# alexnodeland/fugue

Measured on AMD Instinct MI355X. Metric: hmc_leapfrog_steps_per_sec, higher is better.
Workload: dtype f64; 1 GPU; C2-normal32: hmc_chain, 32-site conjugate Normal (x#i~N(0,1), y#i~N(x#i,0.5)=0.2i-1), 65536 chains/GPU, L=16, HMCConfig::default; chains_per_gpu=65536, chains_total=65536, n_leapfrog=16, transitions_per_launch=25

## Files before the change

fugue_amd/build.py:

```python
from __future__ import annotations

import hashlib
import os
import subprocess
import sys
from concurrent.futures import ThreadPoolExecutor

HERE = os.path.dirname(os.path.abspath(__file__))
CSRC = os.path.join(HERE, "csrc")
LIB_DIR = os.path.join(HERE, "lib")
LIB = os.environ.get("FG_LIB_PATH") or os.path.join(LIB_DIR, "libfugue_amd.so")
OBJ_DIR = os.path.join(LIB_DIR, "obj")
SOURCES = ["fg_program.cpp", "fg_dsl.cpp", "fg_diag_host.cpp", "fg_jit.cpp", "fg_engine.hip", "fg_hmc_sep.hip", "fg_hmc_lin.hip", "fg_hmc_interp.hip", "fg_mh.hip", "fg_mh_interp.hip", "fg_smc.hip", "fg_diag.hip", "fg_diag_stream.hip", "fg_diag_qstream.hip", "fg_diag_cstream.hip", "fg_loglik_stream.hip", "fg_state.hip", "fg_vi.hip", "fg_result.hip", "fg_predict.hip", "fg_abc.hip", "fg_rng_debug.hip"]
HEADERS = ["fg_ir.h", "fg_math.h", "fg_interp.h", "fg_program.h", "fg_engine_internal.h", "fg_diag_internal.h", "fg_gradstream.h", "fg_cold.h", "fg_dev_types.h", "fg_jit.h",
           "fg_switch.h", "fg_div2.h", "fg_hmc_sep_plan.h", "fg_mh_mw_plan.h", "fg_hmc_split_plan.h", "fg_diag_qstream_plan.h", "fg_diag_cstream_plan.h", "fg_loglik_stream_plan.h", "fg_result_plan.h", "fg_predict_plan.h", "fg_abc_plan.h", "fg_smc_plan.h", "fg_hmc_jit_body.h", "fg_mh_interp_body.h", "fg_mh_mw_body.h", "fg_mh_mw2_body.h",
           os.path.join("..", "..", "include", "fugue_amd.h")]
FLAGS = ["-O3", "-std=c++17", "-fPIC", "--offload-arch=gfx950", "-ffp-contract=off", "-fno-fast-math", "-DFG_BUILD", "-Wall",
         "-Wno-unused-function"]
LINK_LIBS = []


JIT_HEAD = ["fg_ir.h", "fg_math.h", "fg_cold.h", "fg_dev_types.h"]
JIT_BODIES = {"FG_JIT_EMBED_HMC_BODY": "fg_hmc_jit_body.h", "FG_JIT_EMBED_MH_BODY": "fg_mh_interp_body.h", "FG_JIT_EMBED_INTERP": "fg_interp.h",
              "FG_JIT_EMBED_GRADSTREAM": "fg_gradstream.h", "FG_JIT_EMBED_MHMW_BODY": "fg_mh_mw_body.h", "FG_JIT_EMBED_MHMW2_BODY": "fg_mh_mw2_body.h",
              "FG_JIT_EMBED_API": os.path.join("..", "..", "include", "fugue_amd.h")}


def _write_jit_embed():
    def text(name):
        lines = open(os.path.join(CSRC, name)).read().splitlines()
# ... 127 lines not shown
```

fugue_amd/csrc/fg_dev_types.h:

```cpp
#pragma once
#include "fg_ir.h"

struct FgChainCtx {
    long long C;
    uint32_t chain0;
    unsigned long long seed;
    long long *values;
    double *gtile;
    int gtile_rows;
};


struct FgHmcDev {
    double *lj, *eps, *frozen, *da_mu, *da_leb, *da_hbar;
    unsigned long long *da_m;
    double *m_inv, *mass_sqrt, *w_mean, *w_m2;
    unsigned long long *w_n;
    double *alpha_sum; unsigned long long *n_div;
    double *p0_scratch;
    int L; double h, target; int grad_mode; int use_mass;
    double div2_hi, div2_lo; int div2;
};


__device__ __forceinline__ double fg_kinetic(const FgProgramDev &P, const double *pl, int tw, const double *m_inv, long long C) {
    double s = 0.0;
    if (m_inv) {
        for (int i = 0; i < P.d; ++i) { const double p = pl[i * tw]; s += p * p * m_inv[(long long)i * C]; }
    } else {
#pragma unroll 8
        for (int i = 0; i < P.d; ++i) { const double p = pl[i * tw]; s += p * p; }
    }
    return 0.5 * s;
}


// ... 44 lines not shown
```

fugue_amd/csrc/fg_engine.hip:

```cpp
#include "fg_engine_internal.h"
#include "fg_hmc_sep_plan.h"
#include "fg_div2.h"
#include "fg_gradstream.h"
#include "fg_cold.h"

template <bool GT>
__global__ __launch_bounds__(FG_WAVE, FG_MIN_WAVES) void k_prior_init(FgProgramDev P, FgChainCtx X, uint32_t iteration, uint32_t purpose,
                                                        double *acc_out , double *lj_out ) {
    extern __shared__ double lds_[];
    double *lds = GT ? X.gtile + (size_t)blockIdx.x * X.gtile_rows * FG_WAVE : lds_;
    constexpr int tw = FG_WAVE;
    const long long chain = (long long)blockIdx.x * tw + threadIdx.x;
    const bool live = chain < X.C;
    const long long c = live ? chain : X.C - 1;
    double *slots = lds + threadIdx.x;
    for (int j = 0; j < P.n_slots; ++j) slots[j * tw] = 0.0;
    FgStream rng = fg_stream(X.seed, X.chain0 + (uint32_t)c, iteration, purpose);
    FgAcc3 A = {0.0, 0.0, 0.0};
    fg_exec<FG_MODE_PRIOR, false>(P.ins, P.n_ins, P.pool, slots, tw, A, &rng, nullptr, 0, live);
    if (live) {
        fg_store_values(P, X, c, slots, tw);
        if (acc_out) { acc_out[c] = A.prior; acc_out[X.C + c] = A.lik; acc_out[2 * X.C + c] = A.fac; }
        if (lj_out) lj_out[c] = fg_total(A);
    }
// ... 809 lines not shown
            return FG_E_HIP;
    }
    if (mass && !e->H.m_inv) {
        if (A(&e->H.m_inv, d * C) || A(&e->H.mass_sqrt, d * C) || A(&e->H.w_mean, d * C) || A(&e->H.w_m2, d * C) || A(&e->H.w_n, C))
            return FG_E_HIP;
    }
    return FG_OK;
}

void fg_internal_hmc_set_cfg(fg_engine *e, const fg_hmc_config *cfg) {
    e->cfg = *cfg;
    e->H.L = cfg->n_leapfrog > 1 ? cfg->n_leapfrog : 1;
    e->H.h = cfg->finite_diff_eps; e->H.target = cfg->target_accept;
    e->H.grad_mode = cfg->grad_mode;
    e->H.div2 = fg_div2_prove(2.0 * e->H.h, &e->H.div2_hi, &e->H.div2_lo) ? 1 : 0;
}

static bool hmc_jit_first(const fg_engine *e) {
    const FgJitFirstIn in = { e->cfg.grad_mode, e->jit_state, e->P.gstream != nullptr, e->gt, e->tw, fg_hmc_sep_gate(e->gt, e->P.sep != nullptr, e->sep_disabled, e->d), fg_hmc_lin_gate(e) };
    return fg_hmc_jit_first(in);
}

static int hmc_find_eps(fg_engine *e, uint32_t instance, int injected, double *d_eps_out) {
    if (hmc_jit_first(e)) {
        const int rc = fg_hmc_jit_find_eps(e, instance, injected, d_eps_out);
        if (rc != FG_E_UNSUPPORTED) return rc;
    }
    FG_LAUNCH_GT(e, k_hmc_find_eps, dim3((unsigned)((e->C + e->tw - 1) / e->tw)), dim3(e->tw), e->lds_bytes, e->stream, e->P, e->X, e->H, instance,
                       injected, d_eps_out);
    HIPCHK(hipGetLastError());
// ... 228 lines not shown
    HIPCHK(hipGetLastError());
    e->n_warmup = std::min(e->n_warmup, e->iter);
    if (e->mass_adapt_at >= e->iter) e->mass_adapt_at = -1;
    return FG_OK;
}
int fg_hmc_set_n_leapfrog(fg_engine *e, int n_leapfrog) {
    NEED_ENGINE(e);
    if (!e->hmc_ready) return FG_E_STATE;
    e->cfg.n_leapfrog = n_leapfrog > 1 ? n_leapfrog : 1;
    e->H.L = e->cfg.n_leapfrog;
    return FG_OK;
}
const char *fg_hmc_last_kernel(const fg_engine *e) { return e ? e->last_hmc_kernel.c_str() : ""; }
const char *fg_mh_last_kernel(const fg_engine *e) { return e ? e->last_mh_kernel.c_str() : ""; }
int fg_hmc_short_quotient(const fg_engine *e) { return (e && e->hmc_ready && e->H.div2) ? 1 : 0; }
int fg_hmc_is_warming_up(const fg_engine *e) { return (e && e->hmc_ready && e->iter < e->n_warmup) ? 1 : 0; }
int64_t fg_hmc_iterations(const fg_engine *e) { return (e && e->hmc_ready) ? (int64_t)e->iter : 0; }

int fg_hmc_grad(fg_engine *e, double h, int grad_mode, double *h_grad, int32_t *h_ok) {
    NEED_ENGINE(e);
    if (!h_grad) return FG_E_BAD_ARG;
    if (int rc = hmc_lds_ok(e)) return rc;
    if (grad_mode == FG_GRAD_ANALYTIC && (!e->P.gstream || fg_program_stream_records(e->prog, 2) > 1)) {
        fg_set_error("FG_GRAD_ANALYTIC is not available for this program"); return FG_E_UNSUPPORTED; }
    double *d_g = nullptr;
    int rc = dev_alloc(&d_g, (size_t)std::max(1, e->d) * e->C);
    if (rc) return rc;
    FG_LAUNCH_GT(e, k_hmc_grad, dim3((unsigned)((e->C + e->tw - 1) / e->tw)), dim3(e->tw), e->lds_bytes, e->stream, e->P, e->X, h,
                       grad_mode == FG_GRAD_ANALYTIC ? 2 : (grad_mode == FG_GRAD_FD_SPARSE ? 1 : 0), d_g, e->d_itmp);
    hipError_t le = hipGetLastError();
// ... 213 lines not shown
```

fugue_amd/csrc/fg_hmc_sep.hip:

```cpp
#include "fg_engine_internal.h"
#include "fg_gradstream.h"
#define FG_COLD_UKEY 1
#include "fg_cold.h"
#include "fg_hmc_sep_plan.h"

static_assert(FG_SEP_WAVE == FG_WAVE, "fg_hmc_sep_plan.h sizes tiles for 64-lane waves");

#ifdef FG_HMC_PROF
__device__ unsigned long long fg_hmc_prof[FG_SEP_WMAX][8];
#define FG_PROF_T(i) { const unsigned long long now_ = __builtin_readcyclecounter(); prof_[i] += now_ - tprev_; tprev_ = now_; }
#else
#define FG_PROF_T(i)
#endif
#ifndef FG_SEP_STAGGER
#define FG_SEP_STAGGER 2
#endif

__device__ __forceinline__ fg_u32x8 fg_sep_ld8(const FG_AS4 char *p) { return *(const FG_AS4 fg_u32x8 *)p; }
__device__ __forceinline__ fg_u32x4 fg_sep_ld4(const FG_AS4 char *p) { return *(const FG_AS4 fg_u32x4 *)p; }
__device__ __forceinline__ fg_u32x8 fg_sep_ld8(const char *p) { return *(const fg_u32x8 *)p; }
__device__ __forceinline__ fg_u32x4 fg_sep_ld4(const char *p) { return *(const fg_u32x4 *)p; }
#define FG_SEP_LOAD(k) \
    const fg_u32x8 a##k = fg_sep_ld8(rb + 64 * k); \
    const fg_u32x4 b##k = fg_sep_ld4(rb + 64 * k + 32);
// ... 20 lines not shown
    { const double c = fg_dbl(a##k[2], a##k[3]); const double zp = FG_SEP_Z(k, qp - c), zm = FG_SEP_Z(k, qm - c); \
      outp = FG_SEP_LPF(k, zp); outm = FG_SEP_LPF(k, zm); }
#define FG_SEP_DUALS(k, outp, outm)                                                                    \
    double outp, outm;                                                                                 \
    { const double c = fg_dbl(a##k[2], a##k[3]); const double dp = qp - c, dm = qm - c;                \
      outp = __builtin_fma(nhs2_##k, dp * dp, -fg_dbl(a##k[6], a##k[7])) - 0.5 * FG_LN_2PI;            \
      outm = __builtin_fma(nhs2_##k, dm * dm, -fg_dbl(a##k[6], a##k[7])) - 0.5 * FG_LN_2PI; }
#define FG_SEPD_OWN(k, outp, outm) double outp, outm;                                                  \
    { const double c_ = fg_dbl(a##k[2], a##k[3]); const double zp_ = FG_SEP_Z(k, qp - c_), zm_ = FG_SEP_Z(k, qm - c_); \
      const double lp_ = FG_SEP_LP(k, zp_), lm_ = FG_SEP_LP(k, zm_);                                    \
      outp = (zp_ != zp_) ? FG_NEG_INF : lp_; outm = (zm_ != zm_) ? FG_NEG_INF : lm_; }

template <typename RB> struct FgSepScalarRb { static constexpr bool value = false; };
template <> struct FgSepScalarRb<const FG_AS4 char *> { static constexpr bool value = true; };

template <int NOBS, bool P2, bool CHECK, bool AN = false, bool U0 = false, bool FOLD = false, typename RB = const FG_AS4 char *>
__device__ __forceinline__ bool fg_sep_trajectory(RB rb, double &q_io, double &p_io, double emi, double hk, int L, double h, double two_h,
                                                  double rcp_2h, double *terms, int tw, int nobs_rt, double c_hi = 0.0, double c_lo = 0.0) {
#define FG_SEP_HAS(k) (NOBS >= 0 ? NOBS >= (k) : nobs_rt >= (k))
    FG_SEP_LOAD(0) FG_SEP_LOAD(1) FG_SEP_LOAD(2) FG_SEP_LOAD(3)
    double q = q_io, p = p_io;
    bool bad = false;
    constexpr bool FOLDED = FOLD && P2 && !CHECK && !AN;
    double nhs2_0 = 0.0, nhs2_1 = 0.0, nhs2_2 = 0.0, nhs2_3 = 0.0;
#define FG_SEP_NHS2(k) if (FOLDED && (k > 0 || !U0) && FG_SEP_HAS(k)) { nhs2_##k = fg_dbl(b##k[2], b##k[3]); asm volatile("" : "+v"(nhs2_##k)); }
    FG_SEP_NHS2(0) FG_SEP_NHS2(1) FG_SEP_NHS2(2) FG_SEP_NHS2(3)
#undef FG_SEP_NHS2
    if (FOLD && !CHECK && !AN && FgSepScalarRb<RB>::value) asm volatile("" : "+s"(h), "+s"(c_hi), "+s"(c_lo));
    uint32_t nrange = 0u;
    for (int gs = 0; gs <= L; ++gs) {
        double g;
        if (AN) {
#define FG_SEP_ANTERM(k) { const double dl = q - fg_dbl(a##k[2], a##k[3]);                                                   \
        const double w = (P2 || (a##k[0] & FG_G_POW2)) ? (dl * fg_dbl(a##k[4], a##k[5])) * fg_dbl(a##k[4], a##k[5])         \
                                                       : (dl / fg_dbl(b##k[0], b##k[1])) / fg_dbl(b##k[0], b##k[1]); g = g - w; }
            g = 0.0;
            FG_SEP_ANTERM(0)
            if (FG_SEP_HAS(1)) FG_SEP_ANTERM(1)
            if (FG_SEP_HAS(2)) FG_SEP_ANTERM(2)
            if (FG_SEP_HAS(3)) FG_SEP_ANTERM(3)
#undef FG_SEP_ANTERM
        } else {
        const double qp = q + h, qm = q - h;
        double tp, tm;
        if (FOLDED) {
// ... 18 lines not shown
            }
        } else {
        if (U0) { tp = FG_SEP_LP_U(qp); tm = FG_SEP_LP_U(qm); }
        else { FG_SEP_DUAL(0, tp_, tm_) tp = tp_; tm = tm_; }
        if (FG_SEP_HAS(1)) {
            FG_SEP_DUAL(1, lp1, lm1)
            double sp = lp1, sm = lm1;
            if (FG_SEP_HAS(2)) { FG_SEP_DUAL(2, lp2, lm2) sp += lp2; sm += lm2; }
            if (FG_SEP_HAS(3)) { FG_SEP_DUAL(3, lp3, lm3) sp += lp3; sm += lm3; }
            tp = tp + sp; tm = tm + sm;
        }
        }
        const double n = tp - tm;
        if (!CHECK && FOLD) g = __builtin_fma(n, c_hi, n * c_lo);
        else g = fg_div_const(n, two_h, rcp_2h);
        if (!CHECK && FOLD) {
            uint32_t hi = (uint32_t)__double2hiint(n);
            asm("" : "+v"(hi));
            const uint32_t nr = (hi << 1) - 0x19000000u;
            nrange = nrange > nr ? nrange : nr;
        } else {
        const double an = __builtin_fabs(n);
        if (__builtin_expect(__any(!(an >= 0x1p-823 && an <= 0x1p953)), 0)) g = n / two_h;
        }
        }
        if (CHECK) bad = bad || !fg_finite(g);
        const double kick = hk * g;
        p = p + kick;
        if (gs > 0 && gs < L) { asm volatile(""); p = p + kick; }
        if (gs < L) { asm volatile(""); q = q + emi * p; }
    }
    if (!CHECK && FOLD && nrange >= 0xde000000u) p = __builtin_nan("");
    if (U0) { double lp = FG_SEP_LP_U(q); FG_SEP_NAN_NEG_INF(q, lp) terms[a0[1] * tw] = lp; }
    else FG_SEP_TERM(0)
    if (FG_SEP_HAS(1)) FG_SEP_TERM(1)
    if (FG_SEP_HAS(2)) FG_SEP_TERM(2)
    if (FG_SEP_HAS(3)) FG_SEP_TERM(3)
    q_io = q; p_io = p;
    return bad;
#undef FG_SEP_HAS
}

template <bool AN, typename RB>
__device__ __noinline__ FgD3 fg_sep_trajectory_checked(RB rb, double q, double p, double emi, double hk, int L, double h,
                                                       double two_h, double rcp_2h, double *terms, int tw, int nobs) {
    const bool bad = fg_sep_trajectory<-1, false, true, AN, false, false, RB>(rb, q, p, emi, hk, L, h, two_h, rcp_2h, terms, tw, nobs);
    FgD3 r; r.a = q; r.b = p; r.c = bad ? 1.0 : 0.0;
// ... 95 lines not shown
            double pj = p[j] + hk * g;
            if (gs > 0 && gs < L) pj = pj + hk * g;
            p[j] = pj;
            if (gs < L) q[j] = q[j] + (MASS ? e * mii[j] : e) * pj;
        }
    }
#pragma unroll
    for (int j = 0; j < NC; ++j) {
        if (live) H.p0_scratch[(long long)ci[j] * X.C + c] = q[j];
        kin0[(long long)ci[j] * tw] = k0v[j];
        kin1[(long long)ci[j] * tw] = MASS ? p[j] * p[j] * mii[j] : p[j] * p[j];
    }
    return bad;
}

template <bool MASS, int MODE, int HALF = 0 , int NC = 0, int NOBS_R = 0, bool U0_R = false, bool FOLD = false>
__global__ __launch_bounds__(FG_WAVE * FG_SEP_WMAX, 4) void k_hmc_sep_steps(FgProgramDev P, FgChainCtx X, FgHmcDev H, FgSegSep seg, int iter0, int n_steps,
                                                                             int n_warmup, int welford_on, double *draws, int first_sample_t,
                                                                             double *pos_all , double *info ) {
    extern __shared__ double lds[];
    constexpr int tw = FG_WAVE >> HALF;
    constexpr bool DFAST = MODE == 3, DENSE = MODE == 1 || DFAST, AN = MODE == 2;
    static_assert(!HALF || MODE == 0, "half tiles: sparse finite difference only");
    constexpr bool RES = NC > 0;
    constexpr int NCX = RES ? NC : 1;
    static_assert(!RES || (MODE == 0 && HALF == 0 && NC <= 4 && NOBS_R >= 0 && NOBS_R <= 3), "resident form: sparse 64-chain tiles");
    static_assert(!FOLD || MODE == 0, "the folded trajectory loop: sparse finite difference only");
    const int lane = threadIdx.x & (tw - 1);
    const int half = HALF == 1 ? (int)((threadIdx.x >> 5) & 1u) : (HALF == 2 ? (int)((threadIdx.x >> 4) & 3u) : 0);
    const int wv = __builtin_amdgcn_readfirstlane((int)(threadIdx.x >> 6));
    const long long chain = (long long)blockIdx.x * tw + lane;
    const bool live = chain < X.C;
    const bool live0 = live && half == 0;
    const long long c = live ? chain : X.C - 1;
    const int d = P.d, L = H.L, n_s = P.n_sstream, n_pri = P.n_prior_terms;
    const int srows = P.n_sep_free > 0 ? P.n_slots : 0;
    double *slots = lds + lane;
    double *terms = lds + (long long)(srows + (DENSE ? 0 : 2 * d)) * tw + lane;
    double *xch = terms + (long long)n_s * tw;
    double *qrow = xch + 3 * tw, *prow = qrow + (long long)d * tw;
    double *kin0 = DENSE ? qrow : lds + (long long)srows * tw + lane;
    double *kin1 = DENSE ? prow : kin0 + (long long)d * tw;
// ... 71 lines not shown
#pragma unroll
            for (int j = 0; j < NCX; ++j) {
                if (j >= nown) break;
                const int i = k0 + j;
                if (prio_turns) { if ((j ^ (wv >> 2)) & 1) __builtin_amdgcn_s_setprio(1); else __builtin_amdgcn_s_setprio(0); }
                double z;
                if (!(j & 1)) { const FgD2 zz = have_pre ? zn[j >> 1] : fg_cold_normal_pair(sk0, sk1, gchain, (uint32_t)(i >> 1), (uint32_t)iter, FG_RNG_HMC); z = zz.a; zb = zz.b; }
                else z = zb;
                double p = MASS ? z * msr[j] : z;
                const double mii = mir[j];
                kin0R[i * tw] = MASS ? p * p * mii : p * p;
                double q = qc[j];
                const double emi = MASS ? e * mii : e;
                const double q0 = q, p0 = p;
                const FG_AS4 char *rb = (const FG_AS4 char *)(uintptr_t)(P.sep + roff[j]);
                fg_sep_trajectory<NOBS_R, true, false, false, U0_R, FOLD>(rb, q, p, emi, hk, L, h, two_h, rcp_2h, termsR, tw, NOBS_R, c_hi, c_lo);
                if (__builtin_expect(__any(!fg_finite(p)), 0)) {
                    q = q0; p = p0;
                    FG_SEP_2H(th, rc)
                    bad = fg_sep_trajectory<NOBS_R, true, true, false, U0_R>(rb, q, p, emi, hk, L, h, th, rc, termsR, tw, NOBS_R) || bad;
                }
                qpr[j] = q;
                kin1R[i * tw] = MASS ? p * p * mii : p * p;
            }
        } else if (DFAST) {
            const int own[4] = { seg.own[wv][0], seg.own[wv][1], seg.own[wv][2], seg.own[wv][3] };
#define FG_DENSE_CALL(NC_, OBS_) fg_dense_trajectory<NC_, OBS_, MASS>(P, X, H, own, terms, qrow, kin0, kin1, tw, n_pri, n_s, L, e, h, two_h, rcp_2h, sk0, sk1, gchain, (uint32_t)iter, c, live)
            const int nown = seg.n_own[wv];
            if (n_s > n_pri) { if (nown == 4) bad = FG_DENSE_CALL(4, true); else if (nown == 3) bad = FG_DENSE_CALL(3, true); else if (nown == 2) bad = FG_DENSE_CALL(2, true); else bad = FG_DENSE_CALL(1, true); }
            else { if (nown == 4) bad = FG_DENSE_CALL(4, false); else if (nown == 3) bad = FG_DENSE_CALL(3, false); else if (nown == 2) bad = FG_DENSE_CALL(2, false); else bad = FG_DENSE_CALL(1, false); }
#undef FG_DENSE_CALL
// ... 101 lines not shown
                }
            }
            else if (!(i & 1)) { const FgD2 zz = (HALF != 0 && i == k0 && have_pre) ? zpre : fg_cold_normal_pair(sk0, sk1, gchain, (uint32_t)(i >> 1), (uint32_t)iter, FG_RNG_HMC); z = zz.a; zb = zz.b; }
            else z = zb;
            double p = MASS ? z * ms[(long long)ci * X.C] : z;
            const double mii = MASS ? mi[(long long)ci * X.C] : 1.0;
            if (on) kin0[ci * tw] = MASS ? p * p * mii : p * p;
            const long long gq = (long long)P.f64_site[ci] * X.C + c;
            double q = fg_as_double(X.values[gq]);
            const double emi = MASS ? e * mii : e;
            const FgSepCoord cd = P.sep_coord[i];
            const int nobs = (cd.n & 7) - 1;
            const double q0 = q, p0 = p;
            if (HALF) {
                const char *rb = (const char *)(P.sep + P.sep_coord[ci].off);
#define FG_SEP_CALLH(NO, UU) fg_sep_trajectory<NO, true, false, false, UU, FOLD, const char *>(rb, q, p, emi, hk, L, h, two_h, rcp_2h, terms, tw, NO, c_hi, c_lo)
                if ((cd.n & 512) && nobs == 1) FG_SEP_CALLH(1, true);
                else if (nobs == 1) FG_SEP_CALLH(1, false); else if (nobs == 0) FG_SEP_CALLH(0, false); else if (nobs == 2) FG_SEP_CALLH(2, false); else FG_SEP_CALLH(3, false);
#undef FG_SEP_CALLH
                if (__builtin_expect(__any(!fg_finite(p)), 0)) {
                    FG_SEP_2H(th, rc)
                    const FgD3 r = fg_sep_trajectory_checked<AN, const char *>(rb, q0, p0, emi, hk, L, h, th, rc, terms, tw, nobs);
                    q = r.a; p = r.b; bad = bad || (on && r.c != 0.0);
                }
            } else {
            const FG_AS4 char *rb = (const FG_AS4 char *)(uintptr_t)(P.sep + cd.off);
#define FG_SEP_CALL(NO, PP) fg_sep_trajectory<NO, PP, false, AN, false, FOLD>(rb, q, p, emi, hk, L, h, two_h, rcp_2h, terms, tw, NO, c_hi, c_lo)
            if (!AN && (cd.n & 512) && nobs == 1) fg_sep_trajectory<1, true, false, false, true, FOLD>(rb, q, p, emi, hk, L, h, two_h, rcp_2h, terms, tw, 1, c_hi, c_lo);
            else if (cd.n & 256) { if (nobs == 1) FG_SEP_CALL(1, true); else if (nobs == 0) FG_SEP_CALL(0, true); else if (nobs == 2) FG_SEP_CALL(2, true); else FG_SEP_CALL(3, true); }
            else { if (nobs == 1) FG_SEP_CALL(1, false); else if (nobs == 0) FG_SEP_CALL(0, false); else if (nobs == 2) FG_SEP_CALL(2, false); else FG_SEP_CALL(3, false); }
#undef FG_SEP_CALL
            if (__builtin_expect(__any(!fg_finite(p)), 0)) {
                FG_SEP_2H(th, rc)
                const FgD3 r = fg_sep_trajectory_checked<AN, const FG_AS4 char *>(rb, q0, p0, emi, hk, L, h, th, rc, terms, tw, nobs);
                q = r.a; p = r.b; bad = bad || r.c != 0.0;
            }
            }
            if (live && on) H.p0_scratch[(long long)ci * X.C + c] = q;
            if (on) kin1[ci * tw] = MASS ? p * p * mii : p * p;
        }
        if (bad) atomicOr((unsigned long long *)(xch + 2 * tw), 1ull);
        if (prio_turns) { if (wv == 0) __builtin_amdgcn_s_setprio(2); else __builtin_amdgcn_s_setprio(0); }
        FG_PROF_T(0)
// ... 115 lines not shown
    if (blockIdx.x == 0 && lane == 0) for (int q = 0; q < 8; ++q) fg_hmc_prof[wv][q] = prof_[q];
#endif
    if (RES && live) {
#pragma unroll
        for (int j = 0; j < NCX; ++j)
            if (j < nown) X.values[(long long)P.f64_site[k0 + j] * X.C + c] = fg_as_i64(qc[j]);
    }
    if (wv == 0 && live0) {
        H.lj[c] = lj; H.eps[c] = eps; H.frozen[c] = frozen;
        H.da_mu[c] = da_mu; H.da_leb[c] = da_leb; H.da_hbar[c] = da_hbar; H.da_m[c] = da_m;
        H.alpha_sum[c] += asum; H.n_div[c] += ndiv;
    }
}

using FgSepKernel = void (*)(FgProgramDev, FgChainCtx, FgHmcDev, FgSegSep, int, int, int, int, double *, int, double *, double *);
struct FgSepVariant { FgSepKey key; FgSepKernel fn; unsigned long long raised; };
#define FG_SEP_ENTRY(M, MODE, HALF, NC, NOBS, U0, FOLD) { { M, MODE, HALF, NC, NOBS, U0, FOLD }, k_hmc_sep_steps<M, MODE, HALF, NC, NOBS, U0, FOLD>, 0 },
static FgSepVariant fg_sep_variants[] = { FG_SEP_VARIANTS(FG_SEP_ENTRY) };
#undef FG_SEP_ENTRY

int fg_hmc_sep_launch(fg_engine *e, int iter0, int n, int welford_on, double *draws, int first_sample_t, double *pos_all, double *info) {
    if (!fg_hmc_sep_gate(e->gt, e->P.sep != nullptr, e->sep_disabled, e->d)) return FG_E_UNSUPPORTED;
    const FgSepPlanIn in = { e->C, e->d, e->n_simd, e->n_slots, e->P.n_sep_free, e->P.n_sstream, e->cfg.grad_mode, e->H.use_mass != 0, e->mw_override,
                             e->gt, e->sep_disabled, e->sep_res_disabled, e->sep_fold_disabled, e->prog->sep_fold && e->H.div2 != 0 , &e->prog->sep_coord, &e->prog->sep,
                             fg_env_switch("FG_HMC_SEP_HALF"), fg_env_switch("FG_HMC_DENSE_FAST"), fg_env_switch("FG_HMC_SUM4"), fg_env_switch("FG_HMC_PRIO"),
                             fg_env_switch("FG_HMC_STAGGER"), fg_env_switch("FG_HMC_PREDRAW") };
    FgSepPlan pl;
    int rc = fg_hmc_sep_plan(in, &pl);
    if (rc != FG_OK) return rc;
    FgSepVariant *v = std::find_if(std::begin(fg_sep_variants), std::end(fg_sep_variants), [&](const FgSepVariant &q) { return q.key == pl.key; });
    if (v == std::end(fg_sep_variants)) return FG_E_UNSUPPORTED;
    rc = fg_launch(e, v->fn, v->raised, dim3(pl.tiles), dim3(FG_WAVE * pl.W), pl.lds, e->P, e->X, e->H, pl.seg, iter0, n, e->n_warmup, welford_on, draws, first_sample_t, pos_all, info);
    if (rc == FG_OK) e->last_hmc_kernel = pl.name;
    return rc;
}

#ifdef FG_HMC_PROF
extern "C" int fg_debug_hmc_prof(unsigned long long *out) {
    return hipMemcpyFromSymbol(out, HIP_SYMBOL(fg_hmc_prof), sizeof(unsigned long long) * FG_SEP_WMAX * 8) == hipSuccess ? 0 : -1;
}
#endif
```

fugue_amd/engine.py:

```python
from __future__ import annotations

import ctypes as C
import os
from typing import List, Optional, Sequence

import numpy as np

from . import model as M

_HERE = os.path.dirname(os.path.abspath(__file__))
LIB_PATH = os.environ.get("FG_LIB_PATH") or os.path.join(_HERE, "lib", "libfugue_amd.so")


class fg_tok(C.Structure):
    _fields_ = [("op", C.c_int32), ("a", C.c_int32), ("b", C.c_int32), ("reserved", C.c_int32), ("imm", C.c_double)]


class fg_hmc_config(C.Structure):
    _fields_ = [("n_leapfrog", C.c_int32), ("target_accept", C.c_double), ("init_step_size", C.c_double),
                ("finite_diff_eps", C.c_double), ("adapt_mass", C.c_int32), ("grad_mode", C.c_int32)]


class fg_hmc_stats(C.Structure):
    _fields_ = [("accept_rate", C.c_double), ("mean_step_size", C.c_double), ("n_divergent", C.c_int64),
# ... 35 lines not shown
TOK = {"const": 0, "site": 1, "data": 2, "neg": 3, "exp": 4, "ln": 5, "sqrt": 6, "abs": 7, "floor": 8, "sin": 9,
       "cos": 10, "tanh": 11, "add": 12, "sub": 13, "mul": 14, "div": 15, "pow": 16, "min": 17, "max": 18,
       "clamp": 19, "select": 20}
GRAD_FD_DENSE, GRAD_FD_SPARSE, GRAD_ANALYTIC = 0, 1, 2
FG_E_NO_DEVICE, FG_E_HIP, FG_E_BAD_ARG, FG_E_NOT_FINALIZED, FG_E_STATE, FG_E_UNSUPPORTED, FG_E_LIMIT = -1, -2, -3, -4, -5, -6, -7

ABI_SYMBOLS = [
    "fg_program_new", "fg_program_free", "fg_program_data", "fg_program_sample", "fg_program_observe",
    "fg_program_factor", "fg_program_finalize", "fg_program_n_sites", "fg_program_n_f64", "fg_program_n_observe",
    "fg_program_n_instructions", "fg_program_n_slots", "fg_program_site_name", "fg_program_site_vtype",
    "fg_program_site_of_handle", "fg_program_f64_site", "fg_program_dep_count", "fg_program_stream_records", "fg_last_error", "fg_abi_version",
    "fg_engine_new", "fg_engine_free", "fg_engine_synchronize", "fg_engine_stream", "fg_engine_set_stream", "fg_engine_n_chains",
    "fg_engine_set_values", "fg_engine_get_values", "fg_engine_values_device", "fg_prior_init", "fg_log_joint", "fg_log_joint_stream",
    "fg_program_sample_discrete_uniform",
    "fg_hmc_config_default", "fg_hmc_init", "fg_hmc_step", "fg_hmc_step_info", "fg_hmc_get_mass", "fg_hmc_run", "fg_hmc_get_stats", "fg_hmc_get_step_sizes",
    "fg_hmc_get_log_joint", "fg_hmc_set_step_size", "fg_hmc_set_n_leapfrog", "fg_hmc_is_warming_up", "fg_hmc_iterations", "fg_hmc_short_quotient", "fg_hmc_step_recorded",
    "fg_state_size", "fg_state_export", "fg_state_import", "fg_hmc_grad", "fg_hmc_transition_injected",
    "fg_hmc_find_eps_injected", "fg_mh_init", "fg_mh_step", "fg_mh_set_recording", "fg_mh_run", "fg_mh_get_stats", "fg_mh_get_scales",
    "fg_mh_get_log_weight", "fg_smc_config_default", "fg_smc_run", "fg_smc_prior_particles", "fg_smc_normalize", "fg_smc_ess", "fg_smc_resample", "fg_smc_rejuvenate",
    "fg_smc_get_weights", "fg_smc_set_log_weights", "fg_device_log_sum_exp", "fg_device_next_beta", "fg_device_smc_temper",
    "fg_device_resample_indices", "fg_diag_chain_moments", "fg_diag_autocov_sums", "fg_diag_rhat_ess", "fg_diag_combine", "fg_diag_geweke",
    "fg_diag_combine_reduced", "fg_diag_set_exchange", "fg_diag_exchange_bytes", "fg_hmc_last_kernel", "fg_mh_last_kernel", "fg_diag_quantiles",
    "fg_comm_unique_id", "fg_comm_init", "fg_comm_destroy", "fg_device_alloc", "fg_device_free", "fg_device_download", "fg_device_upload",
    "fg_dsl_compile", "fg_dsl_warning_count", "fg_dsl_warning",
    "fg_vi_config_default", "fg_vi_elbo_batch", "fg_vi_optimize", "fg_vi_estimate_elbo",
    "fg_diag_stream_new", "fg_diag_stream_update", "fg_diag_stream_count", "fg_diag_stream_moments", "fg_diag_stream_autocov_sums",
    "fg_diag_stream_rhat_ess", "fg_diag_stream_free",
    "fg_diag_qstream_new", "fg_diag_qstream_update", "fg_diag_qstream_count", "fg_diag_qstream_end_pass", "fg_diag_qstream_passes",
    "fg_diag_qstream_result", "fg_diag_qstream_free",
    "fg_diag_cstream_new", "fg_diag_cstream_update", "fg_diag_cstream_count", "fg_diag_cstream_result", "fg_diag_cstream_free",
    "fg_diag_cells_f64",
# ... 89 lines not shown
    L.fg_hmc_config_default.argtypes = [C.POINTER(fg_hmc_config)]
    L.fg_hmc_init.argtypes = [vp, C.POINTER(fg_hmc_config), C.c_int]
    L.fg_hmc_step.argtypes = [vp, C.c_int, vp]
    L.fg_hmc_step_info.argtypes = [vp, C.c_int, vp, vp]
    L.fg_hmc_get_mass.argtypes = [vp, dp]
    L.fg_hmc_run.argtypes = [vp, C.POINTER(fg_hmc_config), C.c_int, C.c_int, vp, C.POINTER(fg_hmc_stats)]
    L.fg_hmc_get_stats.argtypes = [vp, C.POINTER(fg_hmc_stats)]
    L.fg_hmc_get_step_sizes.argtypes = [vp, dp]
    L.fg_hmc_get_log_joint.argtypes = [vp, dp]
    L.fg_hmc_set_step_size.argtypes = [vp, C.c_double]
    L.fg_hmc_set_n_leapfrog.argtypes = [vp, C.c_int]
    L.fg_hmc_is_warming_up.argtypes = [vp]
    L.fg_hmc_iterations.restype = C.c_int64
    L.fg_hmc_iterations.argtypes = [vp]
    L.fg_hmc_short_quotient.argtypes = [vp]
    L.fg_hmc_step_recorded.argtypes = [vp, C.c_int, C.POINTER(C.c_int64), dp, dp, ip, vp]
    L.fg_state_size.restype = C.c_int64
    L.fg_state_size.argtypes = [vp]
    L.fg_state_export.argtypes = [vp, vp, C.c_size_t]
    L.fg_state_import.argtypes = [vp, vp, C.c_size_t]
    L.fg_hmc_grad.argtypes = [vp, C.c_double, C.c_int, dp, ip]
    L.fg_hmc_transition_injected.argtypes = [vp, C.POINTER(fg_hmc_config), C.c_double, dp, dp, ip, dp, ip, dp]
    L.fg_hmc_find_eps_injected.argtypes = [vp, C.POINTER(fg_hmc_config), dp, dp]
    L.fg_mh_init.argtypes = [vp, C.c_int, C.POINTER(fg_site_proposal)]
    L.fg_mh_step.argtypes = [vp, C.c_int, ip, C.c_int, vp]
    L.fg_mh_set_recording.argtypes = [vp, C.c_int]
    L.fg_mh_run.argtypes = [vp, C.c_int, C.c_int, C.POINTER(fg_site_proposal), ip, C.c_int, vp, C.POINTER(fg_mh_stats)]
    L.fg_mh_get_stats.argtypes = [vp, C.POINTER(fg_mh_stats)]
    L.fg_mh_get_scales.argtypes = [vp, dp]
    L.fg_mh_get_log_weight.argtypes = [vp, dp]
# ... 397 lines not shown
    def hmc_set_step_size(self, eps: float):
        _check(lib().fg_hmc_set_step_size(self.h, float(eps)))

    def hmc_set_n_leapfrog(self, n: int):
        _check(lib().fg_hmc_set_n_leapfrog(self.h, int(n)))

    def hmc_is_warming_up(self) -> bool:
        return bool(lib().fg_hmc_is_warming_up(self.h))

    def hmc_iterations(self) -> int:
        return int(lib().fg_hmc_iterations(self.h))

    def hmc_short_quotient(self) -> bool:
        return bool(lib().fg_hmc_short_quotient(self.h))

    def hmc_step_recorded(self, chain_ids: Sequence[int], n_leapfrog: int):
        ids = np.ascontiguousarray(chain_ids, dtype=np.int64)
        K, L = ids.size, int(n_leapfrog)
        traj, ham = np.zeros((max(1, K), L + 1, max(1, self.d))), np.zeros((max(1, K), L + 1))
        npts = np.zeros(max(1, K), dtype=np.int32)
        _check(lib().fg_hmc_step_recorded(self.h, K, ids.ctypes.data_as(C.POINTER(C.c_int64)), _dp(traj), _dp(ham),
                                          npts.ctypes.data_as(C.POINTER(C.c_int32)), None))
        return traj[:K, :, :self.d], ham[:K], npts[:K]

    def state_export(self) -> bytes:
        n = lib().fg_state_size(self.h)
        buf = C.create_string_buffer(n)
        _check(lib().fg_state_export(self.h, buf, n))
        return buf.raw

# ... 565 lines not shown
```

include/fugue_amd.h:

```cpp
#ifndef FUGUE_AMD_H
#define FUGUE_AMD_H

#include <stddef.h>
#include <stdint.h>

#ifdef __cplusplus
extern "C" {
#endif

#define FG_ABI_VERSION 1

enum {
    FG_OK = 0,
    FG_E_NO_DEVICE = -1,
    FG_E_HIP = -2,
    FG_E_BAD_ARG = -3,
    FG_E_NOT_FINALIZED = -4,
    FG_E_STATE = -5,
    FG_E_UNSUPPORTED = -6,
    FG_E_LIMIT = -7
};
enum {
    FG_ERR_INVALID_MEAN = 100, FG_ERR_INVALID_VARIANCE = 101, FG_ERR_INVALID_PROBABILITY = 102, FG_ERR_INVALID_SHAPE = 104, FG_ERR_INVALID_COUNT = 106,
    FG_ERR_ADDRESS_CONFLICT = 301, FG_ERR_UNEXPECTED_STRUCTURE = 302,
// ... 118 lines not shown
void fg_hmc_config_default(fg_hmc_config *cfg);
int fg_hmc_init(fg_engine *e, const fg_hmc_config *cfg, int n_warmup);
int fg_hmc_step(fg_engine *e, int n_transitions, double *d_draws);
int fg_hmc_step_info(fg_engine *e, int n_transitions, double *d_positions, double *d_info);
int fg_hmc_run(fg_engine *e, const fg_hmc_config *cfg, int n_samples, int n_warmup,
               double *d_draws, fg_hmc_stats *h_stats);
int fg_hmc_get_stats(fg_engine *e, fg_hmc_stats *h_stats);
int fg_hmc_get_step_sizes(fg_engine *e, double *h_eps );
int fg_hmc_get_log_joint(fg_engine *e, double *h_lj );
int fg_hmc_get_mass(fg_engine *e, double *h_m_inv);
int fg_hmc_set_step_size(fg_engine *e, double eps);
int     fg_hmc_set_n_leapfrog(fg_engine *e, int n_leapfrog);
int     fg_hmc_is_warming_up(const fg_engine *e);
int64_t fg_hmc_iterations(const fg_engine *e);
int     fg_hmc_short_quotient(const fg_engine *e);
const char *fg_hmc_last_kernel(const fg_engine *e);
const char *fg_mh_last_kernel(const fg_engine *e);
int fg_hmc_step_recorded(fg_engine *e, int n_recorded, const int64_t *h_chain_ids, double *h_traj, double *h_ham,
                         int32_t *h_n_points, double *d_info);
int fg_hmc_grad(fg_engine *e, double h, int grad_mode, double *h_grad, int32_t *h_ok);
int fg_hmc_transition_injected(fg_engine *e, const fg_hmc_config *cfg, double eps,
                               const double *h_p0, const double *h_u, int32_t *h_accepted,
                               double *h_alpha, int32_t *h_divergent, double *h_lj);
int fg_hmc_find_eps_injected(fg_engine *e, const fg_hmc_config *cfg, const double *h_p0,
                             double *h_eps);

enum { FG_PROP_AUTO = 0,
       FG_PROP_GAUSSIAN = 1, FG_PROP_LOGSPACE = 2, FG_PROP_REFLECT = 3, FG_PROP_PRIOR_RESAMPLE = 4 };
typedef struct fg_site_proposal {
    int32_t kind; double lower, upper;
// ... 134 lines not shown
```

rust/fugue-gpu/src/ffi.rs:

```rust
#![allow(non_camel_case_types, dead_code)]
use std::os::raw::{c_char, c_int, c_void};

#[repr(C)] pub struct fg_program { _p: [u8; 0] }
#[repr(C)] pub struct fg_engine { _p: [u8; 0] }
#[repr(C)] pub struct fg_diag_stream { _p: [u8; 0] }
#[repr(C)] pub struct fg_diag_qstream { _p: [u8; 0] }
#[repr(C)] pub struct fg_diag_cstream { _p: [u8; 0] }
#[repr(C)] pub struct fg_loglik_stream { _p: [u8; 0] }
#[repr(C)] pub struct fg_abc { _p: [u8; 0] }

pub const FG_E_NO_DEVICE: c_int = -1;
pub const FG_E_HIP: c_int = -2;
pub const FG_E_BAD_ARG: c_int = -3;
pub const FG_E_STATE: c_int = -5;
pub const FG_E_UNSUPPORTED: c_int = -6;
pub const FG_E_LIMIT: c_int = -7;

pub const FG_T_CONST: i32 = 0;
pub const FG_T_SITE: i32 = 1;
pub const FG_T_ADD: i32 = 12;
pub const FG_T_MUL: i32 = 14;
pub const FG_T_SELECT: i32 = 20;

pub const FG_F64: c_int = 0;
// ... 91 lines not shown
                                 h_log_prior: *const f64, h_log_denom: *const f64) -> c_int;
    pub fn fg_hmc_config_default(cfg: *mut fg_hmc_config);
    pub fn fg_hmc_init(e: *mut fg_engine, cfg: *const fg_hmc_config, n_warmup: c_int) -> c_int;
    pub fn fg_hmc_step(e: *mut fg_engine, n: c_int, d_draws: *mut f64) -> c_int;
    pub fn fg_hmc_step_info(e: *mut fg_engine, n: c_int, d_positions: *mut f64, d_info: *mut f64) -> c_int;
    pub fn fg_hmc_step_recorded(e: *mut fg_engine, n_recorded: c_int, h_chain_ids: *const i64, h_traj: *mut f64, h_ham: *mut f64,
                                h_n_points: *mut i32, d_info: *mut f64) -> c_int;
    pub fn fg_hmc_run(e: *mut fg_engine, cfg: *const fg_hmc_config, n_samples: c_int, n_warmup: c_int, d_draws: *mut f64, stats: *mut fg_hmc_stats) -> c_int;
    pub fn fg_hmc_get_stats(e: *mut fg_engine, stats: *mut fg_hmc_stats) -> c_int;
    pub fn fg_hmc_get_step_sizes(e: *mut fg_engine, h_eps: *mut f64) -> c_int;
    pub fn fg_hmc_set_step_size(e: *mut fg_engine, eps: f64) -> c_int;
    pub fn fg_hmc_set_n_leapfrog(e: *mut fg_engine, n_leapfrog: c_int) -> c_int;
    pub fn fg_hmc_is_warming_up(e: *const fg_engine) -> c_int;
    pub fn fg_hmc_iterations(e: *const fg_engine) -> i64;
    pub fn fg_hmc_short_quotient(e: *const fg_engine) -> c_int;
    pub fn fg_hmc_last_kernel(e: *const fg_engine) -> *const c_char;
    pub fn fg_mh_last_kernel(e: *const fg_engine) -> *const c_char;
    pub fn fg_mh_init(e: *mut fg_engine, n_warmup: c_int, overrides: *const fg_site_proposal) -> c_int;
    pub fn fg_mh_step(e: *mut fg_engine, n: c_int, rec_sites: *const i32, n_rec: c_int, d_draws: *mut c_void) -> c_int;
    pub fn fg_mh_set_recording(e: *mut fg_engine, during_adaptation: c_int) -> c_int;
    pub fn fg_mh_run(e: *mut fg_engine, n_samples: c_int, n_warmup: c_int, overrides: *const fg_site_proposal, rec_sites: *const i32, n_rec: c_int,
                     d_draws: *mut c_void, stats: *mut fg_mh_stats) -> c_int;
    pub fn fg_smc_config_default(cfg: *mut fg_smc_config);
    pub fn fg_smc_run(e: *mut fg_engine, cfg: *const fg_smc_config, h_log_w: *mut f64, h_weights: *mut f64, res: *mut fg_smc_result,
                      h_betas: *mut f64, max_betas: c_int) -> c_int;
    pub fn fg_smc_prior_particles(e: *mut fg_engine, iteration: u32) -> c_int;
    pub fn fg_smc_normalize(e: *mut fg_engine) -> c_int;
    pub fn fg_smc_ess(e: *mut fg_engine, out: *mut f64) -> c_int;
    pub fn fg_smc_resample(e: *mut fg_engine, method: c_int, step: u32, h_indices: *mut i64) -> c_int;
    pub fn fg_smc_rejuvenate(e: *mut fg_engine, beta: f64, steps: c_int, first_move_id: u32, h_accept_rate: *mut f64) -> c_int;
// ... 95 lines not shown
```

Baseline: 27.41 billion leapfrog-steps/s.

## Prove finite-difference range on host and skip per-step overflow check in folded HMC

Adds a host-side proof that, for the program's separable Normal records and finite-difference step, the numerator of the folded gradient cannot overflow. When the proof holds, a RANGED kernel variant is launched that drops the per-gradient exponent tracking and the final NaN injection. The leapfrog loop is also peeled into first, middle and last iterations so the per-step branches on gs disappear. This adds a second compiled variant per folded kernel and relies on the bound being sound; an environment switch can turn it off.

```diff
diff --git a/fugue_amd/build.py b/fugue_amd/build.py
--- a/fugue_amd/build.py
+++ b/fugue_amd/build.py
@@ -13,7 +13,7 @@
 OBJ_DIR = os.path.join(LIB_DIR, "obj")
 SOURCES = ["fg_program.cpp", "fg_dsl.cpp", "fg_diag_host.cpp", "fg_jit.cpp", "fg_engine.hip", "fg_hmc_sep.hip", "fg_hmc_lin.hip", "fg_hmc_interp.hip", "fg_mh.hip", "fg_mh_interp.hip", "fg_smc.hip", "fg_diag.hip", "fg_diag_stream.hip", "fg_diag_qstream.hip", "fg_diag_cstream.hip", "fg_loglik_stream.hip", "fg_state.hip", "fg_vi.hip", "fg_result.hip", "fg_predict.hip", "fg_abc.hip", "fg_rng_debug.hip"]
 HEADERS = ["fg_ir.h", "fg_math.h", "fg_interp.h", "fg_program.h", "fg_engine_internal.h", "fg_diag_internal.h", "fg_gradstream.h", "fg_cold.h", "fg_dev_types.h", "fg_jit.h",
-           "fg_switch.h", "fg_div2.h", "fg_hmc_sep_plan.h", "fg_mh_mw_plan.h", "fg_hmc_split_plan.h", "fg_diag_qstream_plan.h", "fg_diag_cstream_plan.h", "fg_loglik_stream_plan.h", "fg_result_plan.h", "fg_predict_plan.h", "fg_abc_plan.h", "fg_smc_plan.h", "fg_hmc_jit_body.h", "fg_mh_interp_body.h", "fg_mh_mw_body.h", "fg_mh_mw2_body.h",
+           "fg_switch.h", "fg_div2.h", "fg_sep_range.h", "fg_hmc_sep_plan.h", "fg_mh_mw_plan.h", "fg_hmc_split_plan.h", "fg_diag_qstream_plan.h", "fg_diag_cstream_plan.h", "fg_loglik_stream_plan.h", "fg_result_plan.h", "fg_predict_plan.h", "fg_abc_plan.h", "fg_smc_plan.h", "fg_hmc_jit_body.h", "fg_mh_interp_body.h", "fg_mh_mw_body.h", "fg_mh_mw2_body.h",
            os.path.join("..", "..", "include", "fugue_amd.h")]
 FLAGS = ["-O3", "-std=c++17", "-fPIC", "--offload-arch=gfx950", "-ffp-contract=off", "-fno-fast-math", "-DFG_BUILD", "-Wall",
          "-Wno-unused-function"]
diff --git a/fugue_amd/csrc/fg_dev_types.h b/fugue_amd/csrc/fg_dev_types.h
--- a/fugue_amd/csrc/fg_dev_types.h
+++ b/fugue_amd/csrc/fg_dev_types.h
@@ -20,6 +20,7 @@
     double *p0_scratch;
     int L; double h, target; int grad_mode; int use_mass;
     double div2_hi, div2_lo; int div2;
+    int range;
 };
 
 
diff --git a/fugue_amd/csrc/fg_engine.hip b/fugue_amd/csrc/fg_engine.hip
--- a/fugue_amd/csrc/fg_engine.hip
+++ b/fugue_amd/csrc/fg_engine.hip
@@ -1,6 +1,7 @@
 #include "fg_engine_internal.h"
 #include "fg_hmc_sep_plan.h"
 #include "fg_div2.h"
+#include "fg_sep_range.h"
 #include "fg_gradstream.h"
 #include "fg_cold.h"
 
@@ -847,6 +848,13 @@
     e->H.h = cfg->finite_diff_eps; e->H.target = cfg->target_accept;
     e->H.grad_mode = cfg->grad_mode;
     e->H.div2 = fg_div2_prove(2.0 * e->H.h, &e->H.div2_hi, &e->H.div2_lo) ? 1 : 0;
+    e->H.range = 0;
+    if (e->prog && !e->prog->sep_coord.empty()) {
+        std::vector<int> off, n; std::vector<double> c, s, lns;
+        for (const FgSepCoord &cd : e->prog->sep_coord) { off.push_back(cd.off); n.push_back(cd.n & 7); }
+        for (const FgSepRec &r : e->prog->sep) { c.push_back(r.c); s.push_back(r.inv); lns.push_back(r.lns); }
+        e->H.range = fg_sep_range_prove(e->H.h, off.size(), off.data(), n.data(), c.data(), s.data(), lns.data(), nullptr) ? 1 : 0;
+    }
 }
 
 static bool hmc_jit_first(const fg_engine *e) {
@@ -1105,6 +1113,7 @@
 const char *fg_hmc_last_kernel(const fg_engine *e) { return e ? e->last_hmc_kernel.c_str() : ""; }
 const char *fg_mh_last_kernel(const fg_engine *e) { return e ? e->last_mh_kernel.c_str() : ""; }
 int fg_hmc_short_quotient(const fg_engine *e) { return (e && e->hmc_ready && e->H.div2) ? 1 : 0; }
+int fg_hmc_range_proved(const fg_engine *e) { return (e && e->hmc_ready && e->H.range) ? 1 : 0; }
 int fg_hmc_is_warming_up(const fg_engine *e) { return (e && e->hmc_ready && e->iter < e->n_warmup) ? 1 : 0; }
 int64_t fg_hmc_iterations(const fg_engine *e) { return (e && e->hmc_ready) ? (int64_t)e->iter : 0; }
 
diff --git a/fugue_amd/csrc/fg_hmc_sep.hip b/fugue_amd/csrc/fg_hmc_sep.hip
--- a/fugue_amd/csrc/fg_hmc_sep.hip
+++ b/fugue_amd/csrc/fg_hmc_sep.hip
@@ -58,7 +58,7 @@
 template <typename RB> struct FgSepScalarRb { static constexpr bool value = false; };
 template <> struct FgSepScalarRb<const FG_AS4 char *> { static constexpr bool value = true; };
 
-template <int NOBS, bool P2, bool CHECK, bool AN = false, bool U0 = false, bool FOLD = false, typename RB = const FG_AS4 char *>
+template <int NOBS, bool P2, bool CHECK, bool AN = false, bool U0 = false, bool FOLD = false, typename RB = const FG_AS4 char *, bool RANGED = false>
 __device__ __forceinline__ bool fg_sep_trajectory(RB rb, double &q_io, double &p_io, double emi, double hk, int L, double h, double two_h,
                                                   double rcp_2h, double *terms, int tw, int nobs_rt, double c_hi = 0.0, double c_lo = 0.0) {
 #define FG_SEP_HAS(k) (NOBS >= 0 ? NOBS >= (k) : nobs_rt >= (k))
@@ -71,8 +71,9 @@
     FG_SEP_NHS2(0) FG_SEP_NHS2(1) FG_SEP_NHS2(2) FG_SEP_NHS2(3)
 #undef FG_SEP_NHS2
     if (FOLD && !CHECK && !AN && FgSepScalarRb<RB>::value) asm volatile("" : "+s"(h), "+s"(c_hi), "+s"(c_lo));
+    if (CHECK && !AN && NOBS >= 0 && FgSepScalarRb<RB>::value) asm volatile("" : "+s"(h));
     uint32_t nrange = 0u;
-    for (int gs = 0; gs <= L; ++gs) {
+    auto grad = [&]() __attribute__((always_inline)) -> double {
         double g;
         if (AN) {
 #define FG_SEP_ANTERM(k) { const double dl = q - fg_dbl(a##k[2], a##k[3]);                                                   \
@@ -121,7 +122,8 @@
         const double n = tp - tm;
         if (!CHECK && FOLD) g = __builtin_fma(n, c_hi, n * c_lo);
         else g = fg_div_const(n, two_h, rcp_2h);
-        if (!CHECK && FOLD) {
+        if (!CHECK && FOLD && RANGED) {
+        } else if (!CHECK && FOLD) {
             uint32_t hi = (uint32_t)__double2hiint(n);
             asm("" : "+v"(hi));
             const uint32_t nr = (hi << 1) - 0x19000000u;
@@ -132,12 +134,17 @@
         }
         }
         if (CHECK) bad = bad || !fg_finite(g);
-        const double kick = hk * g;
+        return g;
+    };
+    { const double kick = hk * grad(); p = p + kick; asm volatile(""); q = q + emi * p; }
+    for (int gs = 1; gs < L; ++gs) {
+        const double kick = hk * grad();
         p = p + kick;
-        if (gs > 0 && gs < L) { asm volatile(""); p = p + kick; }
-        if (gs < L) { asm volatile(""); q = q + emi * p; }
-    }
-    if (!CHECK && FOLD && nrange >= 0xde000000u) p = __builtin_nan("");
+        asm volatile(""); p = p + kick;
+        asm volatile(""); q = q + emi * p;
+    }
+    { const double kick = hk * grad(); p = p + kick; }
+    if (!CHECK && FOLD && !RANGED && nrange >= 0xde000000u) p = __builtin_nan("");
     if (U0) { double lp = FG_SEP_LP_U(q); FG_SEP_NAN_NEG_INF(q, lp) terms[a0[1] * tw] = lp; }
     else FG_SEP_TERM(0)
     if (FG_SEP_HAS(1)) FG_SEP_TERM(1)
@@ -263,7 +270,8 @@
     return bad;
 }
 
-template <bool MASS, int MODE, int HALF = 0 , int NC = 0, int NOBS_R = 0, bool U0_R = false, bool FOLD = false>
+template <bool MASS, int MODE, int HALF = 0 , int NC = 0, int NOBS_R = 0, bool U0_R = false, bool FOLD = false,
+          bool RANGED = false >
 __global__ __launch_bounds__(FG_WAVE * FG_SEP_WMAX, 4) void k_hmc_sep_steps(FgProgramDev P, FgChainCtx X, FgHmcDev H, FgSegSep seg, int iter0, int n_steps,
                                                                              int n_warmup, int welford_on, double *draws, int first_sample_t,
                                                                              double *pos_all , double *info ) {
@@ -275,6 +283,7 @@
     constexpr int NCX = RES ? NC : 1;
     static_assert(!RES || (MODE == 0 && HALF == 0 && NC <= 4 && NOBS_R >= 0 && NOBS_R <= 3), "resident form: sparse 64-chain tiles");
     static_assert(!FOLD || MODE == 0, "the folded trajectory loop: sparse finite difference only");
+    static_assert(!RANGED || FOLD, "the range test is the folded loop's");
     const int lane = threadIdx.x & (tw - 1);
     const int half = HALF == 1 ? (int)((threadIdx.x >> 5) & 1u) : (HALF == 2 ? (int)((threadIdx.x >> 4) & 3u) : 0);
     const int wv = __builtin_amdgcn_readfirstlane((int)(threadIdx.x >> 6));
@@ -376,7 +385,7 @@
                 const double emi = MASS ? e * mii : e;
                 const double q0 = q, p0 = p;
                 const FG_AS4 char *rb = (const FG_AS4 char *)(uintptr_t)(P.sep + roff[j]);
-                fg_sep_trajectory<NOBS_R, true, false, false, U0_R, FOLD>(rb, q, p, emi, hk, L, h, two_h, rcp_2h, termsR, tw, NOBS_R, c_hi, c_lo);
+                fg_sep_trajectory<NOBS_R, true, false, false, U0_R, FOLD, const FG_AS4 char *, RANGED>(rb, q, p, emi, hk, L, h, two_h, rcp_2h, termsR, tw, NOBS_R, c_hi, c_lo);
                 if (__builtin_expect(__any(!fg_finite(p)), 0)) {
                     q = q0; p = p0;
                     FG_SEP_2H(th, rc)
@@ -508,7 +517,7 @@
             const double q0 = q, p0 = p;
             if (HALF) {
                 const char *rb = (const char *)(P.sep + P.sep_coord[ci].off);
-#define FG_SEP_CALLH(NO, UU) fg_sep_trajectory<NO, true, false, false, UU, FOLD, const char *>(rb, q, p, emi, hk, L, h, two_h, rcp_2h, terms, tw, NO, c_hi, c_lo)
+#define FG_SEP_CALLH(NO, UU) fg_sep_trajectory<NO, true, false, false, UU, FOLD, const char *, RANGED>(rb, q, p, emi, hk, L, h, two_h, rcp_2h, terms, tw, NO, c_hi, c_lo)
                 if ((cd.n & 512) && nobs == 1) FG_SEP_CALLH(1, true);
                 else if (nobs == 1) FG_SEP_CALLH(1, false); else if (nobs == 0) FG_SEP_CALLH(0, false); else if (nobs == 2) FG_SEP_CALLH(2, false); else FG_SEP_CALLH(3, false);
 #undef FG_SEP_CALLH
@@ -519,8 +528,8 @@
                 }
             } else {
             const FG_AS4 char *rb = (const FG_AS4 char *)(uintptr_t)(P.sep + cd.off);
-#define FG_SEP_CALL(NO, PP) fg_sep_trajectory<NO, PP, false, AN, false, FOLD>(rb, q, p, emi, hk, L, h, two_h, rcp_2h, terms, tw, NO, c_hi, c_lo)
-            if (!AN && (cd.n & 512) && nobs == 1) fg_sep_trajectory<1, true, false, false, true, FOLD>(rb, q, p, emi, hk, L, h, two_h, rcp_2h, terms, tw, 1, c_hi, c_lo);
+#define FG_SEP_CALL(NO, PP) fg_sep_trajectory<NO, PP, false, AN, false, FOLD, const FG_AS4 char *, RANGED>(rb, q, p, emi, hk, L, h, two_h, rcp_2h, terms, tw, NO, c_hi, c_lo)
+            if (!AN && (cd.n & 512) && nobs == 1) fg_sep_trajectory<1, true, false, false, true, FOLD, const FG_AS4 char *, RANGED>(rb, q, p, emi, hk, L, h, two_h, rcp_2h, terms, tw, 1, c_hi, c_lo);
             else if (cd.n & 256) { if (nobs == 1) FG_SEP_CALL(1, true); else if (nobs == 0) FG_SEP_CALL(0, true); else if (nobs == 2) FG_SEP_CALL(2, true); else FG_SEP_CALL(3, true); }
             else { if (nobs == 1) FG_SEP_CALL(1, false); else if (nobs == 0) FG_SEP_CALL(0, false); else if (nobs == 2) FG_SEP_CALL(2, false); else FG_SEP_CALL(3, false); }
 #undef FG_SEP_CALL
@@ -666,8 +675,11 @@
 }
 
 using FgSepKernel = void (*)(FgProgramDev, FgChainCtx, FgHmcDev, FgSegSep, int, int, int, int, double *, int, double *, double *);
-struct FgSepVariant { FgSepKey key; FgSepKernel fn; unsigned long long raised; };
-#define FG_SEP_ENTRY(M, MODE, HALF, NC, NOBS, U0, FOLD) { { M, MODE, HALF, NC, NOBS, U0, FOLD }, k_hmc_sep_steps<M, MODE, HALF, NC, NOBS, U0, FOLD>, 0 },
+struct FgSepVariant { FgSepKey key; FgSepKernel fn, fn_ranged; unsigned long long raised, raised_ranged; };
+template <bool M, int MODE, int HALF, int NC, int NOBS, bool U0, bool FOLD> static constexpr FgSepKernel fg_sep_ranged_fn() {
+    if constexpr (FOLD && !(M && HALF == 0 && NC == 0)) return k_hmc_sep_steps<M, MODE, HALF, NC, NOBS, U0, true, true>; else return nullptr;
+}
+#define FG_SEP_ENTRY(M, MODE, HALF, NC, NOBS, U0, FOLD) { { M, MODE, HALF, NC, NOBS, U0, FOLD }, k_hmc_sep_steps<M, MODE, HALF, NC, NOBS, U0, FOLD>, fg_sep_ranged_fn<M, MODE, HALF, NC, NOBS, U0, FOLD>(), 0, 0 },
 static FgSepVariant fg_sep_variants[] = { FG_SEP_VARIANTS(FG_SEP_ENTRY) };
 #undef FG_SEP_ENTRY
 
@@ -682,7 +694,8 @@
     if (rc != FG_OK) return rc;
     FgSepVariant *v = std::find_if(std::begin(fg_sep_variants), std::end(fg_sep_variants), [&](const FgSepVariant &q) { return q.key == pl.key; });
     if (v == std::end(fg_sep_variants)) return FG_E_UNSUPPORTED;
-    rc = fg_launch(e, v->fn, v->raised, dim3(pl.tiles), dim3(FG_WAVE * pl.W), pl.lds, e->P, e->X, e->H, pl.seg, iter0, n, e->n_warmup, welford_on, draws, first_sample_t, pos_all, info);
+    const bool ranged = v->fn_ranged && e->H.range != 0 && !fg_switch_is(fg_env_switch("FG_HMC_SEP_RANGE"), 0);
+    rc = fg_launch(e, ranged ? v->fn_ranged : v->fn, ranged ? v->raised_ranged : v->raised, dim3(pl.tiles), dim3(FG_WAVE * pl.W), pl.lds, e->P, e->X, e->H, pl.seg, iter0, n, e->n_warmup, welford_on, draws, first_sample_t, pos_all, info);
     if (rc == FG_OK) e->last_hmc_kernel = pl.name;
     return rc;
 }
diff --git a/fugue_amd/csrc/fg_sep_range.h b/fugue_amd/csrc/fg_sep_range.h
--- /dev/null
+++ b/fugue_amd/csrc/fg_sep_range.h
@@ -0,0 +1,29 @@
+#pragma once
+#include <cmath>
+#include <cstddef>
+
+#define FG_SEP_RANGE_HALF_LN_2PI 0.91893853320467274178
+
+inline double fg_sep_range_bound(double h, int nrec, const double *c, const double *s, const double *lns) {
+    const double Q = 0x1p55 * h + h;
+    double sum = 0.0;
+    for (int k = 0; k < nrec; ++k) {
+        const double D = Q + std::fabs(c[k]);
+        sum += 0.5 * (s[k] * s[k]) * (D * D) + std::fabs(lns[k]) + FG_SEP_RANGE_HALF_LN_2PI;
+    }
+    return 2.0 * sum * (1.0 + 0x1p-40);
+}
+
+inline bool fg_sep_range_ok(double h, double bound) { return h > 0.0 && std::isfinite(h) && bound < 0x1p953; }
+
+inline bool fg_sep_range_prove(double h, size_t ncoord, const int *off, const int *n, const double *c, const double *s, const double *lns, double *worst) {
+    bool ok = ncoord > 0;
+    double w = 0.0;
+    for (size_t j = 0; j < ncoord; ++j) {
+        const double b = fg_sep_range_bound(h, n[j], c + off[j], s + off[j], lns + off[j]);
+        if (!fg_sep_range_ok(h, b)) ok = false;
+        if (w == w && !(b <= w)) w = b;
+    }
+    if (worst) *worst = w;
+    return ok;
+}
diff --git a/fugue_amd/engine.py b/fugue_amd/engine.py
--- a/fugue_amd/engine.py
+++ b/fugue_amd/engine.py
@@ -73,7 +73,7 @@
     "fg_engine_set_values", "fg_engine_get_values", "fg_engine_values_device", "fg_prior_init", "fg_log_joint", "fg_log_joint_stream",
     "fg_program_sample_discrete_uniform",
     "fg_hmc_config_default", "fg_hmc_init", "fg_hmc_step", "fg_hmc_step_info", "fg_hmc_get_mass", "fg_hmc_run", "fg_hmc_get_stats", "fg_hmc_get_step_sizes",
-    "fg_hmc_get_log_joint", "fg_hmc_set_step_size", "fg_hmc_set_n_leapfrog", "fg_hmc_is_warming_up", "fg_hmc_iterations", "fg_hmc_short_quotient", "fg_hmc_step_recorded",
+    "fg_hmc_get_log_joint", "fg_hmc_set_step_size", "fg_hmc_set_n_leapfrog", "fg_hmc_is_warming_up", "fg_hmc_iterations", "fg_hmc_short_quotient", "fg_hmc_range_proved", "fg_hmc_step_recorded",
     "fg_state_size", "fg_state_export", "fg_state_import", "fg_hmc_grad", "fg_hmc_transition_injected",
     "fg_hmc_find_eps_injected", "fg_mh_init", "fg_mh_step", "fg_mh_set_recording", "fg_mh_run", "fg_mh_get_stats", "fg_mh_get_scales",
     "fg_mh_get_log_weight", "fg_smc_config_default", "fg_smc_run", "fg_smc_prior_particles", "fg_smc_normalize", "fg_smc_ess", "fg_smc_resample", "fg_smc_rejuvenate",
@@ -193,6 +193,7 @@
     L.fg_hmc_iterations.restype = C.c_int64
     L.fg_hmc_iterations.argtypes = [vp]
     L.fg_hmc_short_quotient.argtypes = [vp]
+    L.fg_hmc_range_proved.argtypes = [vp]
     L.fg_hmc_step_recorded.argtypes = [vp, C.c_int, C.POINTER(C.c_int64), dp, dp, ip, vp]
     L.fg_state_size.restype = C.c_int64
     L.fg_state_size.argtypes = [vp]
@@ -620,6 +621,9 @@
     def hmc_short_quotient(self) -> bool:
         return bool(lib().fg_hmc_short_quotient(self.h))
 
+    def hmc_range_proved(self) -> bool:
+        return bool(lib().fg_hmc_range_proved(self.h))
+
     def hmc_step_recorded(self, chain_ids: Sequence[int], n_leapfrog: int):
         ids = np.ascontiguousarray(chain_ids, dtype=np.int64)
         K, L = ids.size, int(n_leapfrog)
diff --git a/include/fugue_amd.h b/include/fugue_amd.h
--- a/include/fugue_amd.h
+++ b/include/fugue_amd.h
@@ -156,6 +156,7 @@
 int     fg_hmc_is_warming_up(const fg_engine *e);
 int64_t fg_hmc_iterations(const fg_engine *e);
 int     fg_hmc_short_quotient(const fg_engine *e);
+int     fg_hmc_range_proved(const fg_engine *e);
 const char *fg_hmc_last_kernel(const fg_engine *e);
 const char *fg_mh_last_kernel(const fg_engine *e);
 int fg_hmc_step_recorded(fg_engine *e, int n_recorded, const int64_t *h_chain_ids, double *h_traj, double *h_ham,
diff --git a/rust/fugue-gpu/src/ffi.rs b/rust/fugue-gpu/src/ffi.rs
--- a/rust/fugue-gpu/src/ffi.rs
+++ b/rust/fugue-gpu/src/ffi.rs
@@ -129,6 +129,7 @@
     pub fn fg_hmc_is_warming_up(e: *const fg_engine) -> c_int;
     pub fn fg_hmc_iterations(e: *const fg_engine) -> i64;
     pub fn fg_hmc_short_quotient(e: *const fg_engine) -> c_int;
+    pub fn fg_hmc_range_proved(e: *const fg_engine) -> c_int;
     pub fn fg_hmc_last_kernel(e: *const fg_engine) -> *const c_char;
     pub fn fg_mh_last_kernel(e: *const fg_engine) -> *const c_char;
     pub fn fg_mh_init(e: *mut fg_engine, n_warmup: c_int, overrides: *const fg_site_proposal) -> c_int;
```

Measured after the change: 29.88 billion leapfrog-steps/s (median of 6 runs). +9.0%, better.
